# frozenreboot/rplidar_ros2_driver

Hardware: AMD Instinct MI355X
Metric: Mpoints/s raw-scan->filtered PointCloud2 (higher is better)
Workload: dtype u32/f32

## Files before the change

rplidar_ros2_driver_amd/csrc/rpl_device.hpp:

```cpp
#pragma once
#include <hip/hip_runtime.h>
#include <stdint.h>

#include "rplgpu.h"

namespace rpl {

constexpr int kBlock = 1024;
constexpr int kWaves = kBlock / 64;
constexpr int kIters = 32;
constexpr uint32_t kMaxN = 32768;
constexpr int kChunks = kIters * kWaves;
constexpr double kTwoPi = 6.283185307179586476925286766559;

struct Tables {
  const float *angle;
  const float *angle_inv;
  const float2 *cs;
  const float2 *cs_inv;
  const double *rcp;
  uint32_t *work_ctr;
  uint32_t n_cu;
  void *voxel_store;
  uint32_t voxel_store_wgs;
  uint32_t voxel_store_recs;
  unsigned long long *voxel_stats;
  unsigned long long *voxel_stats_host;
  int32_t voxel_split;
  const float *scan_t0;
  uint32_t *redo;
};

struct KParams {
  int32_t is_new_protocol;
  int32_t inverted;
  int32_t scan_processing;
  int32_t clip_enable;
  uint32_t q_min;
  float range_min;
  float range_max;
  float voxel_leaf;
  float ror_r2;
  uint32_t ror_k;
  double vox_scale;
  float vox_scale_f;
  int32_t vox_L;
  int32_t vox_bias;
  float inv_leaf;
  float leaf_s;
  float inv_leaf_s;
  uint32_t d_lo;
  uint32_t d_span;
  int32_t cell_range_safe;
  unsigned long long *dbg;
  uint32_t *cell_keys;
  int32_t fast_div;
  int32_t fast_d4000;
};

__device__ __forceinline__ uint32_t nd_q14(uint2 v) { return v.x & 0xFFFFu; }
__device__ __forceinline__ uint32_t nd_dist(uint2 v) {
  return __builtin_amdgcn_alignbit(v.y, v.x, 16);
}
__device__ __forceinline__ uint32_t nd_quality(uint2 v) { return (v.y >> 16) & 0xFFu; }

__device__ __forceinline__ float nd_dist_m(uint32_t dist_q2) {
  return __uint2float_rn(dist_q2) / 4000.0f;
}
__device__ __forceinline__ float nd_intensity(uint32_t quality, int is_new_protocol) {
  return is_new_protocol ? (float)quality : (float)(quality >> 2);
}
__device__ __forceinline__ bool nd_keep(uint32_t dist_q2, uint32_t quality, const KParams &p) {
  bool k = (dist_q2 - p.d_lo) <= p.d_span;
  if (p.clip_enable) k = k && (quality >= p.q_min);
// ... 100 lines not shown
```

rplidar_ros2_driver_amd/csrc/rpl_voxel.hip:

```cpp
#include <algorithm>
#include <cstdlib>
#include <type_traits>

#include "rpl_device.hpp"
#include "rpl_launch.hpp"
#include "rpl_xf.hpp"

namespace rpl {

#ifndef RPL_VOXEL_THREADS
#define RPL_VOXEL_THREADS 1024
#endif
#ifndef RPL_VOXEL_WGS_PER_CU
#define RPL_VOXEL_WGS_PER_CU (RPL_VOXEL_THREADS == 512 ? 2 : 1)
#endif
constexpr int kVB = RPL_VOXEL_THREADS;
constexpr int kVW = kVB / 64;
constexpr int kVWG = RPL_VOXEL_WGS_PER_CU;
constexpr uint32_t kRecCap = kVWG == 2 ? 4096u : 7168u;
constexpr uint32_t kRecPerThread = kRecCap / kVB;
constexpr uint32_t kRowCap = kVWG == 2 ? 1024u : 2u * kVB;
constexpr uint32_t kRowsPerThread = kRowCap / kVB;
constexpr uint32_t kBucketCap = kRecCap + 3u * kRowCap;
constexpr uint32_t kEmptyKey = 0xFFFFFFFFu;
// ... 242 lines not shown
  const u32x4 marker = {kEmptyKey, 0u, 0u, 0u};
  VoxelLds &L = S.L;
  uint4 *const G = S.G;
  const uint32_t lds_rec = (uint32_t)(uintptr_t)&L.rec[0];
  if (base + 1u + total <= kRecCap) {
    if (lane_id() == 0) lds_store128(lds_rec + base * 16u, marker);
#pragma unroll
    for (int j = 0; j < NS; ++j)
      if (__builtin_amdgcn_inverse_ballot_w64(m[j])) lds_store128(lds_rec + pos[j] * 16u, rec[j]);
  } else {
    if (lane_id() == 0) {
      if (base < kRecCap) lds_store128(lds_rec + base * 16u, marker); else glb_store128(G + base, marker);
    }
#pragma unroll
    for (int j = 0; j < NS; ++j) {
      if (__builtin_amdgcn_inverse_ballot_w64(m[j])) {
        if (pos[j] < kRecCap) lds_store128(lds_rec + pos[j] * 16u, rec[j]); else glb_store128(G + pos[j], rec[j]);
      }
    }
  }
  return false;
}

template <int NS>
__device__ __forceinline__ void voxel_block_split(QueueSink &S,
                                                  const bool (&ok)[NS], const uint32_t (&key)[NS],
                                                  const uint32_t (&qx)[NS], const uint32_t (&qy)[NS],
                                                  const uint32_t (&ci)[NS]) {
#pragma unroll
  for (uint32_t cls = 0; cls < 2u; ++cls) {
    bool okc[NS];
    uint32_t keyc[NS], qxc[NS], qyc[NS], cic[NS];
#pragma unroll
    for (int j = 0; j < NS; ++j) {
      okc[j] = ok[j] && (((key[j] >> 16) ^ key[j]) & 1u) == cls;
      keyc[j] = key[j];
      qxc[j] = okc[j] ? qx[j] : 0u;
      qyc[j] = okc[j] ? qy[j] : 0u;
      cic[j] = okc[j] ? ci[j] : 0u;
    }
    voxel_block_pass<true, NS, kPassPlain>(S, okc, keyc, qxc, qyc, cic);
  }
}

__device__ __forceinline__ double run_sum_f64(uint32_t u) {
  double s = (double)u;
  if (u >= 0xF0000000u) s -= 4294967296.0;
  return s;
}

struct VoxelArena {
  float4 *base;
  unsigned long long *cursor;
  unsigned long long capacity;
  unsigned long long *scan_start;
  int xyi;
};
enum : int { kEmitLegacy = 0, kEmitArenaFirst = 1, kEmitCountOnly = 2, kEmitArenaKnown = 3, kEmitArenaTemp = 4 };

template <bool DBG>
struct PhaseClock {
  unsigned long long acc[8] = {0, 0, 0, 0, 0, 0, 0, 0}, mark = 0;
  __device__ __forceinline__ void start() {
    if (DBG) mark = clock64();
  }
  __device__ __forceinline__ void lap(int i) {
    if (DBG) {
      const unsigned long long now = clock64();
      acc[i] += now - mark;
      mark = now;
    }
  }
};

template <bool DBG, bool CELLS>
__device__ __forceinline__ uint32_t voxel_reduce(VoxelLds &L, const KParams &p,
                                                 float4 *__restrict__ out, uint32_t out_stride,
                                                 uint32_t b, uint32_t *ncell_out, int mode,
                                                 const VoxelArena &arena, bool normalised,
                                                 const float4 *out_buffer) {
  PhaseClock<DBG> pc;
  pc.start();
  auto flush_dbg = [&]() {
    if (DBG && p.dbg && threadIdx.x == 0) {
#pragma unroll
      for (int i = 1; i < 8; ++i) atomicAdd(&p.dbg[16 * b + i], pc.acc[i]);
    }
  };
  uint32_t *const rowstart = L.rows, *const rowfill = L.rows + kRowCap;
  uint32_t *cell_keys = p.cell_keys ? p.cell_keys + (out - out_buffer) : nullptr;
  const int vbias = p.vox_bias;
  const uint32_t nrec = L.misc[0];
  if (DBG && p.dbg && threadIdx.x == 0) pc.acc[7] += (unsigned long long)nrec << 40;
  uint4 mine[kRecPerThread];
  uint32_t rmin = 0xFFFFFFFFu, rmax = 0u;
#pragma unroll
  for (int k = 0; k < (int)kRecPerThread; ++k) {
    const uint32_t idx = threadIdx.x + (uint32_t)k * kVB;
    uint4 m = make_uint4(kEmptyKey, 0u, 0u, 0u);
    if ((idx & ~63u) < nrec) {
      const uint4 raw = L.rec[idx];
      const bool ok = idx < nrec && raw.x != kEmptyKey;
      m = raw;
      if (!normalised) {
        uint4 pr;
        pr.y = (uint32_t)__builtin_amdgcn_update_dpp(0, (int)raw.y, 0x138, 0xF, 0xF, false);
// ... 831 lines not shown
        L.misc[7] = 0u;
      }
      __syncthreads();
      arena_at = ((unsigned long long)L.tmp[29] << 32) | L.tmp[28];
      out = arena.base + arena_at;
      emit_mode = kEmitArenaKnown;
    }
    if (emit_mode == kEmitArenaTemp && L.misc[3] == 0u) {
      const uint32_t total = L.misc[7];
      if (threadIdx.x == 0) {
        const unsigned long long at = atomicAdd(arena.cursor, (unsigned long long)total);
        L.tmp[28] = (uint32_t)at;
        L.tmp[29] = (uint32_t)(at >> 32);
      }
      __syncthreads();
      arena_at = ((unsigned long long)L.tmp[29] << 32) | L.tmp[28];
      const unsigned long long room = arena_at >= arena.capacity ? 0ull : arena.capacity - arena_at;
      const uint32_t ncopy = (uint32_t)min((unsigned long long)total, room);
      const float4 *src = reinterpret_cast<const float4 *>(G + T.voxel_store_recs);
      if (arena.xyi) {
        float *dst = reinterpret_cast<float *>(arena.base) + 3u * (size_t)arena_at;
        for (uint32_t i = threadIdx.x; i < ncopy; i += kVB) {
          const float4 v = src[i];
          dst[3u * i] = v.x;
          dst[3u * i + 1u] = v.y;
          dst[3u * i + 2u] = v.w;
        }
      } else {
        float4 *dst = arena.base + arena_at;
        for (uint32_t i = threadIdx.x; i < ncopy; i += kVB) dst[i] = src[i];
      }
    }
  }
  if (DBG && p.dbg && threadIdx.x == 0) {
    atomicAdd(&p.dbg[16 * b], pc.acc[0]);
    atomicAdd(&p.dbg[16 * b + 2], pc.acc[2]);
  }

  if (flags) atomicOr(&L.misc[1], flags);
  __syncthreads();
  if (threadIdx.x == 0 && !abandoned) {
    const uint32_t total = L.misc[7];
    if (arena.base) {
      const unsigned long long room = arena_at >= arena.capacity ? 0ull : arena.capacity - arena_at;
      const uint32_t kept = (uint32_t)min((unsigned long long)total, room);
      arena.scan_start[b] = arena_at;
      n_points[b] = kept;
      if (status) status[b] = L.misc[1] | (kept < total ? RPLGPU_SCAN_OUT_TRUNCATED : 0u);
    } else {
      n_points[b] = min(total, out_stride);
      if (status) status[b] = L.misc[1] | ((total > out_stride) ? RPLGPU_SCAN_OUT_TRUNCATED : 0u);
    }
  }
  if (RORM != 2 && B <= gridDim.x) return;
  if (threadIdx.x == 0) L.tmp[31] = gridDim.x + atomicAdd(&T.work_ctr[0], 1u);
  __syncthreads();
  bl = L.tmp[31];
  __syncthreads();
  }
}

template <bool FAST_DIV, bool SAFE, bool DBG, bool SPLIT, int RORM = 0>
__global__ __launch_bounds__(kVB) __attribute__((amdgpu_waves_per_eu(kVB * kVWG / 256, kVB * kVWG / 256))) void k_cloud_voxel(
    const uint2 *__restrict__ nodes, uint32_t n_stride, const uint32_t *__restrict__ n_per_scan,
    KParams p, Tables T, const uint32_t *__restrict__ keepmask, uint32_t mask_stride,
    float4 *__restrict__ xyzi, uint32_t out_stride, uint32_t *__restrict__ n_points,
    uint32_t *__restrict__ status, uint32_t B, VoxelArena arena, uint4 *__restrict__ store,
    uint32_t group, uint32_t n_scans, const float *__restrict__ motion,
    const float *__restrict__ pose2d) {
  __shared__ VoxelLds L;
  uint4 *G = store + (size_t)blockIdx.x * 2u * T.voxel_store_recs;
  const float2 *cs = p.inverted ? T.cs_inv : T.cs;
  const uint32_t ishift = p.is_new_protocol ? 0u : 2u;
  const uint32_t ibfe_off = 16u + ishift, ibfe_w = 0xFFu >> ishift;
  const uint32_t q_min16 = p.clip_enable ? (min(p.q_min, 256u) << 16) : 0u;
  const bool use_xf = (group > 1u) || motion || pose2d;
  __shared__ RorSide Rs;
  auto phase_s = [&](uint32_t b, uint32_t, uint32_t &flags) -> bool {
    QueueSink sink{L, G};
    const uint32_t s_lo = b * group, s_hi = min(n_scans, s_lo + group);
    for (uint32_t sc = s_lo; sc < s_hi; ++sc) {
      const uint32_t n = (uint32_t)__builtin_amdgcn_readfirstlane(
          (int)min(n_per_scan[sc], min(n_stride, kMaxN)));
      const uint2 *scan = nodes + (size_t)sc * n_stride;
      const __amdgpu_buffer_rsrc_t scan_rsrc =
          __builtin_amdgcn_make_buffer_rsrc((void *)scan, 0, (int)(n * 8u), 0x00020000);
      const ScanSide sd = scan_side(sc, keepmask, mask_stride, motion, pose2d, T.scan_t0);
      const uint32_t blk0 = (uint32_t)__builtin_amdgcn_readfirstlane((int)wave_id());
      if constexpr (RORM == 1) {
        if (threadIdx.x == 0) { Rs.n_todo = 0u; Rs.n_todo2 = 0u; }
        __syncthreads();
        voxel_stream_dispatch<FAST_DIV, SAFE, SPLIT, false, RPL_VOXEL_AHEAD, 1>(
            sink, p, cs, scan_rsrc, blk0, (n + 123u) / 124u, sd, 0u, use_xf, q_min16, ibfe_off, ibfe_w, flags,
            nullptr, &Rs, (n * 8u + 15u) & ~15u);
        asm volatile("s_waitcnt vmcnt(0) lgkmcnt(0)" ::: "memory");
        __syncthreads();
        bool clutter;
        if (use_xf)
          clutter = ror_resolve<FAST_DIV, SAFE, true>(sink, Rs, p, cs, scan, n, sd.xf, q_min16, ibfe_off, ibfe_w, flags);
        else
          clutter = ror_resolve<FAST_DIV, SAFE, false>(sink, Rs, p, cs, scan, n, sd.xf, q_min16, ibfe_off, ibfe_w, flags);
        if (clutter) return true;
        __syncthreads();
      } else {
        voxel_stream_dispatch<FAST_DIV, SAFE, SPLIT, DBG, RPL_VOXEL_AHEAD, RORM>(
            sink, p, cs, scan_rsrc, blk0, (n + 127u) >> 7, sd, mask_stride, use_xf, q_min16, ibfe_off,
            ibfe_w, flags, (DBG && p.dbg) ? p.dbg + 16 * b : nullptr);
      }
    }
    return false;
  };
  voxel_work_loop<DBG, RORM, SPLIT || RORM != 0>(L, p, T, G, xyzi, out_stride, n_points, status, B, 0u, arena, phase_s);
}

__global__ __launch_bounds__(256) void k_validate_div(float d, float rd, uint32_t e_lo,
                                                      uint32_t e_hi, uint32_t *mismatches) {
  const uint64_t per_exp = 1ull << 23;
  const uint64_t total = (uint64_t)(e_hi - e_lo + 1) * per_exp;
  uint32_t bad = 0;
  for (uint64_t t = (uint64_t)blockIdx.x * blockDim.x + threadIdx.x; t < total;
       t += (uint64_t)gridDim.x * blockDim.x) {
    uint32_t bits = ((uint32_t)(e_lo + (uint32_t)(t >> 23)) << 23) | (uint32_t)(t & (per_exp - 1));
    float a = __uint_as_float(bits);
    float na = __uint_as_float(bits | 0x80000000u);
    const f2 q2 = div_by2(f2{a, na}, d, rd);
    bad += (__float_as_uint(q2.x) != __float_as_uint(a / d));
    bad += (__float_as_uint(q2.y) != __float_as_uint(na / d));
    bad += (__float_as_uint(div_by(a, d, rd)) != __float_as_uint(a / d));
  }
  if (blockIdx.x == 0 && threadIdx.x == 0) {
    bad += (div_by(0.0f, d, rd) != 0.0f);
    bad += (div_by(-0.0f, d, rd) != 0.0f);
  }
  if (bad) atomicAdd(mismatches, bad);
}

hipError_t launch_validate_div(hipStream_t s, float d, float rd, uint32_t e_lo, uint32_t e_hi,
                               uint32_t *d_mismatches) {
  hipLaunchKernelGGL(k_validate_div, dim3(256 * 16), dim3(256), 0, s, d, rd, e_lo, e_hi,
                     d_mismatches);
  return hipGetLastError();
}

uint32_t voxel_max_workgroups(uint32_t n_cu) { return (uint32_t)kVWG * (n_cu ? n_cu : 256u); }


hipError_t launch_cloud_voxel(hipStream_t s, const void *nodes, uint32_t n_stride,
                              const uint32_t *n_per_scan, uint32_t B, const KParams &p,
                              const Tables &T, const uint32_t *keepmask, uint32_t mask_stride,
                              float *xyzi, uint32_t out_stride, uint32_t *n_points,
                              uint32_t *status, float *arena, unsigned long long arena_capacity,
                              unsigned long long *arena_cursor, unsigned long long *scan_start,
                              uint32_t group, const float *motion, const float *pose2d,
                              int arena_form, int ror_mode) {
  if (B == 0) return hipSuccess;
  if (ror_mode && (!p.fast_div || !T.redo || p.dbg)) return hipErrorInvalidValue;
  if (ror_mode == 2 && !keepmask) return hipErrorInvalidValue;
  if (arena_form == 2 && !ror_mode && (p.dbg || !T.voxel_split)) return hipErrorInvalidValue;
  if (group == 0) group = 1;
  group = std::min(group, B);
  const uint32_t n_scans = B;
  B = (B + group - 1u) / group;
  if (!T.voxel_store || T.voxel_store_wgs == 0) return hipErrorInvalidValue;
  if (voxel_store_need(group, n_stride) > T.voxel_store_recs) return hipErrorInvalidValue;
  VoxelArena ar;
  ar.base = (float4 *)arena;
  ar.cursor = arena_cursor;
  ar.capacity = arena_capacity;
  ar.scan_start = scan_start;
  ar.xyi = arena ? arena_form : 0;
  if (kVWG == 2 && group > 1) return hipErrorInvalidValue;
  uint32_t grid = std::min<uint32_t>(std::min<uint32_t>(B, voxel_max_workgroups(T.n_cu)),
                                     T.voxel_store_wgs);
  if (const char *e = std::getenv("RPLGPU_VOXEL_GRID")) {
    const long g = std::atol(e);
    if (g > 0) grid = std::min<uint32_t>(grid, (uint32_t)g);
  }
  const bool with_stats = T.voxel_stats && T.voxel_stats_host && B >= 64u && ror_mode != 2;
  Tables Tk = T;
  if (!with_stats) Tk.voxel_stats = nullptr;
  if (with_stats)
    if (hipError_t e = hipMemsetAsync(T.voxel_stats, 0, 16, s); e != hipSuccess) return e;
  if (grid < B || ror_mode == 2)
    if (hipError_t e = hipMemsetAsync(T.work_ctr, 0, 4, s); e != hipSuccess) return e;
#define RPL_LAUNCH_VOXEL(FD, SF, DB, SP)                                                          \
  hipLaunchKernelGGL((k_cloud_voxel<FD, SF, DB, SP>), dim3(grid), dim3(kVB), 0, s, (const uint2 *)nodes, \
                     n_stride, n_per_scan, p, Tk, keepmask, mask_stride, (float4 *)xyzi, out_stride, \
                     n_points, status, B, ar, (uint4 *)T.voxel_store, group, n_scans, motion, pose2d)
#define RPL_LAUNCH_VOXEL_SF(FD, DB, SP)                                                           \
  do {                                                                                             \
    if (p.cell_range_safe) RPL_LAUNCH_VOXEL(FD, true, DB, SP); else RPL_LAUNCH_VOXEL(FD, false, DB, SP); \
  } while (0)
#define RPL_LAUNCH_VOXEL_ROR(SF, SP, RM)                                                          \
  hipLaunchKernelGGL((k_cloud_voxel<true, SF, false, SP, RM>), dim3(grid), dim3(kVB), 0, s,         \
                     (const uint2 *)nodes, n_stride, n_per_scan, p, Tk, keepmask, mask_stride,      \
                     (float4 *)xyzi, out_stride, n_points, status, B, ar, (uint4 *)T.voxel_store,   \
                     group, n_scans, motion, pose2d)
#define RPL_LAUNCH_VOXEL_ROR_SF(SP, RM)                                                           \
  do {                                                                                             \
    if (p.cell_range_safe) RPL_LAUNCH_VOXEL_ROR(true, SP, RM); else RPL_LAUNCH_VOXEL_ROR(false, SP, RM); \
  } while (0)
  if (ror_mode == 1) {
    if (T.voxel_split) RPL_LAUNCH_VOXEL_ROR_SF(true, 1); else RPL_LAUNCH_VOXEL_ROR_SF(false, 1);
  } else if (ror_mode == 2) {
    if (T.voxel_split) RPL_LAUNCH_VOXEL_ROR_SF(true, 2); else RPL_LAUNCH_VOXEL_ROR_SF(false, 2);
  } else
  if (p.dbg) {
    if (p.fast_div) RPL_LAUNCH_VOXEL_SF(true, true, false); else RPL_LAUNCH_VOXEL_SF(false, true, false);
  } else if (T.voxel_split) {
    if (p.fast_div) RPL_LAUNCH_VOXEL_SF(true, false, true); else RPL_LAUNCH_VOXEL_SF(false, false, true);
  } else {
    if (p.fast_div) RPL_LAUNCH_VOXEL_SF(true, false, false); else RPL_LAUNCH_VOXEL_SF(false, false, false);
  }
#undef RPL_LAUNCH_VOXEL_SF
#undef RPL_LAUNCH_VOXEL
#undef RPL_LAUNCH_VOXEL_ROR_SF
#undef RPL_LAUNCH_VOXEL_ROR
  if (with_stats) {
    if (hipError_t e = hipMemcpyAsync(T.voxel_stats_host, T.voxel_stats, 16, hipMemcpyDeviceToHost, s);
        e != hipSuccess)
      return e;
  }
  return hipGetLastError();
}

}
```

rplidar_ros2_driver_amd/csrc/rplgpu_api.hip:

```cpp
#include <hip/hip_runtime.h>
#include <dlfcn.h>

#include <algorithm>
#include <cmath>
#include <cstdio>
#include <cstdlib>
#include <cstring>
#include <limits>
#include <new>
#include <string>
#include <thread>
#include <vector>

#include "rplgpu.h"
#include "rplgpu_msg.h"
#include "rpl_launch.hpp"
#include "rpl_msg.hpp"
#include "rpl_comm_layout.hpp"
#include "rpl_cells.hpp"

struct VoxelBatchId {
  const void *nodes = nullptr;
  uint32_t n_stride = 0, B = 0, group = 0;
  bool operator==(const VoxelBatchId &o) const {
    return nodes == o.nodes && n_stride == o.n_stride && B == o.B && group == o.group;
  }
};

struct rplgpu_ctx {
  int device = -1;
  hipStream_t own_stream = nullptr;
  hipStream_t stream = nullptr;
  uint32_t max_n = 0, max_b = 0;
  float *d_angle = nullptr, *d_angle_inv = nullptr, *d_inc = nullptr, *d_rinc = nullptr;
  float2 *d_cs = nullptr, *d_cs_inv = nullptr;
  double *d_rcp = nullptr;
  unsigned char *h_pin = nullptr;
  unsigned char *d_pin = nullptr;
  bool zero_copy = true;
  bool spin_sync = true;
  size_t flag_off = 0;
  uint32_t scan_seq = 0;
  struct Pinned { unsigned char *host, *dev; size_t bytes; };
  std::vector<Pinned> pinned;
  unsigned char *d_nodes = nullptr, *d_out = nullptr;
  uint32_t *d_rormask = nullptr;
  uint32_t *d_redo = nullptr;
  int32_t ror_fused = 1;
  uint32_t *d_need_sort = nullptr;
  uint32_t need_sort_cap = 0;
  uint32_t *d_small = nullptr;
  bool div4000_ok = false;
  float leaf_checked = 0.0f;
  bool leaf_ok = false;
  bool idx_checked = false, idx_ok = false;
  unsigned long long *dbg = nullptr;
  uint32_t *cell_keys = nullptr;
  const float *scan_t0 = nullptr;
  unsigned long long *h_vstats = nullptr;
  uint32_t stats_group = 1;
  bool stats_valid = false;
  VoxelBatchId stats_id;
  struct VoxelDecision { VoxelBatchId id; bool split = false; bool valid = false; };
  VoxelDecision decisions[8];
  uint32_t next_decision = 0;
  int32_t last_split = 0;
  uint32_t n_cu = 0;
  void *d_vstore = nullptr;
  int32_t force_split = -1;
  bool dec_stage = true;
  uint32_t vstore_wgs = 0;
  uint32_t vstore_recs = 0;
  uint32_t *d_merge = nullptr;
  size_t merge_cap = 0;
  unsigned long long *d_mkeys = nullptr;
  size_t mkeys_cap = 0;
  bool mkeys_clean = true;
  float2 *d_medges = nullptr;
  size_t medges_cap = 0;
  bool mspec_valid = false;
  rplgpu_scan_merge_t mspec;
  rpl::MergeK mspec_k;
  unsigned char *d_dec = nullptr;
  size_t dec_cap = 0;
  unsigned char *d_scans = nullptr;
  size_t scans_cap = 0;
  uint32_t *d_dec_todo = nullptr;
  size_t dec_todo_cap = 0;
  bool check_ptrs = true;
  void *comm = nullptr;
  int32_t comm_rank = 0, comm_world = 0;
  hipStream_t xstream = nullptr;
  hipEvent_t ev_main = nullptr, ev_x[4] = {nullptr, nullptr, nullptr, nullptr};
  uint32_t n_exchanges = 0;
  std::string err;
};

struct rplgpu_nccl_id_t {
  char internal[128];
};

namespace {

constexpr uint32_t kMaskStride = rpl::kMaxN / 32u;
constexpr size_t kTail = 64;

thread_local std::string g_create_err;

#define RPL_HIP(ctx, call)                                                              \
  do {                                                                                  \
    hipError_t e_ = (call);                                                             \
    if (e_ != hipSuccess) {                                                             \
      (ctx)->err = std::string(#call) + ": " + hipGetErrorString(e_);                   \
      return RPLGPU_ERR_HIP;                                                            \
    }                                                                                   \
  } while (0)

inline float host_dist_m(uint32_t d) { return static_cast<float>(d) / 4000.0f; }

bool make_keep_interval(float range_min, float range_max, uint32_t *lo, uint32_t *hi) {
  const uint32_t dmax = 0xFFFFFFFFu;
  if (!(host_dist_m(dmax) >= range_min)) return false;
  if (!(host_dist_m(1u) <= range_max)) return false;
  uint32_t a = 1u, b = dmax;
  while (a < b) {
    uint32_t m = a + (b - a) / 2;
    if (host_dist_m(m) >= range_min) b = m; else a = m + 1;
  }
  *lo = a;
  a = 1u, b = dmax;
  while (a < b) {
    uint32_t m = a + (b - a + 1) / 2;
    if (host_dist_m(m) <= range_max) a = m; else b = m - 1;
  }
  *hi = a;
  return *lo <= *hi;
}

rpl::KParams to_kparams(const rplgpu_params_t &p) {
  rpl::KParams k;
  k.is_new_protocol = p.is_new_protocol != 0;
  k.inverted = p.inverted != 0;
  k.scan_processing = p.scan_processing != 0;
  k.clip_enable = p.clip_enable != 0;
  k.q_min = p.q_min;
  k.range_min = p.range_min;
  k.range_max = p.range_max;
  k.voxel_leaf = p.voxel_leaf;
  k.ror_r2 = p.ror_radius * p.ror_radius;
  k.ror_k = p.ror_min_neighbors;
  k.vox_scale = 1.0;
  k.vox_scale_f = 1.0f;
  k.vox_L = 1;
  k.vox_bias = 0;
  k.inv_leaf = 1.0f;
  k.leaf_s = 1.0f;
  k.inv_leaf_s = 1.0f;
  k.fast_div = 0;
  k.fast_d4000 = 0;
  k.dbg = nullptr;
  k.cell_keys = nullptr;
  k.d_lo = 1u;
  k.d_span = 0xFFFFFFFEu;
  k.cell_range_safe = 0;
  if (k.clip_enable) {
    uint32_t lo, hi;
// ... 14 lines not shown
    k.inv_leaf = 1.0f / p.voxel_leaf;
    k.leaf_s = p.voxel_leaf * k.vox_scale_f;
    k.inv_leaf_s = k.inv_leaf / k.vox_scale_f;
  }
  return k;
}

bool voxel_split_for(rplgpu_ctx *c, const void *d_nodes, uint32_t n_stride, uint32_t B, uint32_t group) {
  group = std::max(1u, std::min(group, std::max(B, 1u)));
  const VoxelBatchId id{d_nodes, n_stride, B, group};
  const bool with_stats = c->h_vstats && (B + group - 1u) / group >= 64u;
  auto find = [&](const VoxelBatchId &k) -> rplgpu_ctx::VoxelDecision * {
    for (auto &d : c->decisions)
      if (d.valid && d.id == k) return &d;
    return nullptr;
  };
  if (c->h_vstats && c->stats_valid) {
    const unsigned long long entries = __atomic_load_n(&c->h_vstats[0], __ATOMIC_RELAXED);
    const unsigned long long items = __atomic_load_n(&c->h_vstats[1], __ATOMIC_RELAXED);
    const uint32_t g = c->stats_group;
    if (items != 0 && entries <= items * g * 70000ull) {
      rplgpu_ctx::VoxelDecision *d = find(c->stats_id);
      if (!d) {
        d = &c->decisions[c->next_decision];
        c->next_decision = (c->next_decision + 1u) % (uint32_t)(sizeof(c->decisions) / sizeof(c->decisions[0]));
        d->id = c->stats_id;
        d->split = false;
        d->valid = true;
      }
      const unsigned long long avg = entries / (items * g);
      if (!d->split && avg > 6500ull) d->split = true;
      else if (d->split && avg < 4000ull) d->split = false;
    }
  }
  const rplgpu_ctx::VoxelDecision *mine = find(id);
  const bool split = mine ? mine->split : false;
  if (with_stats) {
    c->stats_id = id;
    c->stats_valid = true;
    c->stats_group = group;
  }
  c->last_split = (c->force_split >= 0 ? c->force_split != 0 : split) ? 1 : 0;
  return c->last_split != 0;
}

rpl::Tables tables_of(rplgpu_ctx *c) {
  rpl::Tables t;
  t.angle = c->d_angle;
  t.angle_inv = c->d_angle_inv;
  t.cs = c->d_cs;
  t.cs_inv = c->d_cs_inv;
  t.rcp = c->d_rcp;
  t.work_ctr = c->d_small + 16;
  t.n_cu = c->n_cu;
  t.voxel_store = c->d_vstore;
  t.voxel_store_wgs = c->vstore_wgs;
  t.voxel_store_recs = c->vstore_recs;
  t.voxel_stats = reinterpret_cast<unsigned long long *>(c->d_small + 24);
  t.voxel_stats_host = c->h_vstats;
  t.voxel_split = c->force_split > 0 ? 1 : 0;
  t.scan_t0 = c->scan_t0;
  t.redo = c->d_redo;
  return t;
}

void build_tables(std::vector<float> &angle, std::vector<float> &angle_inv,
                  std::vector<float2> &cs, std::vector<float2> &cs_inv, std::vector<float> &inc,
                  std::vector<float> &rinc) {
  angle.resize(65536);
  angle_inv.resize(65536);
  cs.resize(65536);
  cs_inv.resize(65536);
  for (int q = 0; q < 65536; ++q) {
    uint16_t angle_z_q14 = (uint16_t)q;
    float angle_deg = angle_z_q14 * 90.0f / 16384.0f;
    float angle_rad = angle_deg * (M_PI / 180.0f);
    if (angle_rad < 0.0f) angle_rad += 2.0f * M_PI;
    if (angle_rad >= 2.0f * M_PI) angle_rad -= 2.0f * M_PI;
    float inv = (2.0f * M_PI) - angle_rad;
    if (inv >= 2.0f * M_PI) inv -= 2.0f * M_PI;
    angle[q] = angle_rad;
    angle_inv[q] = inv;
    cs[q] = make_float2((float)std::cos((double)angle_rad), (float)std::sin((double)angle_rad));
    cs_inv[q] = make_float2((float)std::cos((double)inv), (float)std::sin((double)inv));
  }
  inc.resize(rpl::kMaxN + 1);
  inc[0] = 0.0f;
  for (uint32_t c = 1; c <= rpl::kMaxN; ++c)
    inc[c] = static_cast<float>((2.0 * M_PI) / static_cast<double>(c));
  rinc.resize(rpl::kMaxN + 1);
  rinc[0] = 0.0f;
  for (uint32_t c = 1; c <= rpl::kMaxN; ++c) rinc[c] = 1.0f / inc[c];
}

template <class T>
int32_t upload(rplgpu_ctx *c, T **dst, const std::vector<T> &src) {
  RPL_HIP(c, hipMalloc((void **)dst, src.size() * sizeof(T)));
  RPL_HIP(c, hipMemcpy(*dst, src.data(), src.size() * sizeof(T), hipMemcpyHostToDevice));
  return RPLGPU_OK;
}

void comm_teardown(rplgpu_ctx *c);

void free_ctx(rplgpu_ctx *c) {
  if (!c) return;
  if (c->device >= 0) (void)hipSetDevice(c->device);
// ... 222 lines not shown
  if (const char *e = std::getenv("RPLGPU_CHECK_POINTERS")) c->check_ptrs = std::atoi(e) != 0;
  auto fail = [&](int32_t code) {
    g_create_err = c->err;
    free_ctx(c);
    return code;
  };
  if (hipStreamCreateWithFlags(&c->own_stream, hipStreamNonBlocking) != hipSuccess)
    return fail(RPLGPU_ERR_HIP);
  c->stream = c->own_stream;

  std::vector<float> angle, angle_inv, inc, rinc;
  std::vector<float2> cs, cs_inv;
  build_tables(angle, angle_inv, cs, cs_inv, inc, rinc);
  for (int q = 1; q < 65536; ++q) {
    if (!(angle[q] > angle[q - 1])) {
      c->err = "angle table not strictly increasing";
      return fail(RPLGPU_ERR_INVALID_ARG);
    }
  }
  std::vector<double> rcp(rpl::kMaxN + 1);
  rcp[0] = 0.0;
  for (uint32_t k = 1; k <= rpl::kMaxN; ++k) rcp[k] = 1.0 / static_cast<double>(k);
  int32_t rc;
  if ((rc = upload(c, &c->d_rcp, rcp)) || (rc = upload(c, &c->d_angle, angle)) || (rc = upload(c, &c->d_angle_inv, angle_inv)) ||
      (rc = upload(c, &c->d_cs, cs)) || (rc = upload(c, &c->d_cs_inv, cs_inv)) ||
      (rc = upload(c, &c->d_inc, inc)) || (rc = upload(c, &c->d_rinc, rinc)))
    return fail(rc);

  const size_t n = c->max_n;
  c->flag_off = n * 8 + n * 16 + 2 * kTail;
  if (hipHostMalloc((void **)&c->h_pin, n * 8 + n * 16 + 3 * kTail, hipHostMallocDefault) != hipSuccess ||
      hipMalloc((void **)&c->d_nodes, n * 8 + kTail) != hipSuccess ||
      hipMalloc((void **)&c->d_out, n * 16 + kTail) != hipSuccess ||
      hipMalloc((void **)&c->d_small, 128) != hipSuccess ||
      hipMalloc((void **)&c->d_need_sort, ((size_t)c->max_b + 1u) * 4u) != hipSuccess ||
      hipMalloc((void **)&c->d_rormask, (size_t)c->max_b * kMaskStride * 4u) != hipSuccess ||
      hipMalloc((void **)&c->d_redo, ((size_t)c->max_b + 4u) * 4u) != hipSuccess) {
    c->err = "staging allocation failed";
    return fail(RPLGPU_ERR_HIP);
  }
  c->need_sort_cap = c->max_b;
  if (hipMemset(c->d_need_sort, 0, 4) != hipSuccess) {
    c->err = "staging allocation failed";
    return fail(RPLGPU_ERR_HIP);
  }
  c->vstore_wgs = std::min<uint32_t>(c->max_b, rpl::voxel_max_workgroups(c->n_cu));
  c->vstore_recs = (uint32_t)rpl::voxel_store_need(1u, rpl::kMaxN);
  if (hipMalloc(&c->d_vstore, (size_t)c->vstore_wgs * c->vstore_recs * 32u) != hipSuccess) {
    c->err = "record store allocation failed";
    return fail(RPLGPU_ERR_HIP);
  }
  if (hipHostMalloc((void **)&c->h_vstats, 16, hipHostMallocDefault) == hipSuccess) {
    c->h_vstats[0] = c->h_vstats[1] = 0ull;
  } else {
    c->h_vstats = nullptr;
    (void)hipGetLastError();
  }
  if (hipHostGetDevicePointer((void **)&c->d_pin, c->h_pin, 0) != hipSuccess) c->d_pin = nullptr;
  if (const char *e = std::getenv("RPLGPU_ZERO_COPY")) c->zero_copy = std::atoi(e) != 0;
  if (!c->d_pin) c->zero_copy = false;
  if (const char *e = std::getenv("RPLGPU_SPIN_SYNC")) c->spin_sync = std::atoi(e) != 0;
  if (const char *e = std::getenv("RPLGPU_DEC_STAGE")) c->dec_stage = std::atoi(e) != 0;
  if (const char *e = std::getenv("RPLGPU_VOXEL_SPLIT")) c->force_split = std::atoi(e) != 0;
  if (const char *e = std::getenv("RPLGPU_ROR_FUSED")) c->ror_fused = std::atoi(e) != 0;
  std::memset(c->h_pin + c->flag_off, 0, kTail);
  if (hipMemset(c->d_small, 0, 128) != hipSuccess) {
    c->err = "staging clear failed";
    return fail(RPLGPU_ERR_HIP);
  }
  if (validate_divisor(c, 4000.0f, 127, 159, &c->div4000_ok) != RPLGPU_OK) return fail(RPLGPU_ERR_HIP);
  if (validate_divisor(c, 0.05f, 27, 167, &c->leaf_ok) != RPLGPU_OK) return fail(RPLGPU_ERR_HIP);
  c->leaf_checked = 0.05f;
  *out = c;
  return RPLGPU_OK;
}

int32_t rplgpu_destroy(rplgpu_handle_t h) {
  if (!h) return RPLGPU_ERR_INVALID_ARG;
  (void)hipSetDevice(h->device);
  (void)hipStreamSynchronize(h->stream);
  free_ctx(h);
  return RPLGPU_OK;
}

const char *rplgpu_last_error(rplgpu_handle_t h) {
  if (!h) return g_create_err.c_str();
  return h->err.c_str();
}

int32_t rplgpu_set_stream(rplgpu_handle_t h, void *hip_stream) {
  if (!h) return RPLGPU_ERR_INVALID_ARG;
  hipStream_t next = hip_stream ? (hipStream_t)hip_stream : h->own_stream;
  if (next != h->stream) {
    RPL_HIP(h, hipSetDevice(h->device));
    RPL_HIP(h, hipStreamSynchronize(h->stream));
  }
  h->stream = next;
  return RPLGPU_OK;
}

int32_t rplgpu_set_cell_key_output(rplgpu_handle_t h, uint32_t *d_cell_keys) {
  if (!h) return RPLGPU_ERR_INVALID_ARG;
  if (d_cell_keys && !device_readable(h, d_cell_keys, "d_cell_keys")) return RPLGPU_ERR_INVALID_ARG;
  h->cell_keys = d_cell_keys;
  return RPLGPU_OK;
}

int32_t rplgpu_set_scan_time_offsets_dev(rplgpu_handle_t h, const float *d_t0) {
  if (!h) return RPLGPU_ERR_INVALID_ARG;
  if (d_t0 && !device_readable(h, d_t0, "d_t0")) return RPLGPU_ERR_INVALID_ARG;
  h->scan_t0 = d_t0;
  return RPLGPU_OK;
}

int32_t rplgpu_set_voxel_aggregation(rplgpu_handle_t h, int32_t mode) {
  if (!h || mode < RPLGPU_VOXEL_AGG_AUTO || mode > RPLGPU_VOXEL_AGG_TWO_CLASS) return RPLGPU_ERR_INVALID_ARG;
  h->force_split = mode == RPLGPU_VOXEL_AGG_AUTO ? -1 : (mode == RPLGPU_VOXEL_AGG_TWO_CLASS ? 1 : 0);
  return RPLGPU_OK;
}

int32_t rplgpu_debug_set_cycle_buffer(rplgpu_handle_t h, void *d_buf) {
  if (!h) return RPLGPU_ERR_INVALID_ARG;
  h->dbg = (unsigned long long *)d_buf;
  return RPLGPU_OK;
}
int32_t rplgpu_debug_ascend_sorted(rplgpu_handle_t h, uint32_t *count) {
  if (!h || !count) return RPLGPU_ERR_INVALID_ARG;
  RPL_HIP(h, hipSetDevice(h->device));
  RPL_HIP(h, hipStreamSynchronize(h->stream));
  RPL_HIP(h, hipMemcpy(count, h->d_small + 28, 4, hipMemcpyDeviceToHost));
  return RPLGPU_OK;
}
int32_t rplgpu_debug_voxel_instance(rplgpu_handle_t h) { return h ? h->last_split : RPLGPU_ERR_INVALID_ARG; }
int32_t rplgpu_set_ror_mode(rplgpu_handle_t h, int32_t mode) {
  if (!h || (mode != RPLGPU_ROR_INSIDE && mode != RPLGPU_ROR_TWO_KERNELS)) return RPLGPU_ERR_INVALID_ARG;
  h->ror_fused = mode == RPLGPU_ROR_INSIDE ? 1 : 0;
  return RPLGPU_OK;
}
int32_t rplgpu_debug_ror_listed(rplgpu_handle_t h, uint32_t *count) {
  if (!h || !count) return RPLGPU_ERR_INVALID_ARG;
  RPL_HIP(h, hipSetDevice(h->device));
  RPL_HIP(h, hipStreamSynchronize(h->stream));
  RPL_HIP(h, hipMemcpy(count, h->d_redo, 4, hipMemcpyDeviceToHost));
  return RPLGPU_OK;
}
int32_t rplgpu_debug_fast_div(rplgpu_handle_t h) {
  if (!h) return RPLGPU_ERR_INVALID_ARG;
  return (h->div4000_ok ? 1 : 0) | (h->leaf_ok ? 2 : 0) | (h->idx_ok ? 4 : 0);
// ... 78 lines not shown
    if (ror_inside && h->ror_fused && p->voxel_enable && kp.fast_div && !kp.dbg) {
      *ror_inside = true;
    } else {
      RPL_HIP(h, rpl::launch_ror_mask(h->stream, d_nodes, n_stride, d_n_per_scan, B, kp,
                                      tables_of(h), h->d_rormask, kMaskStride));
      *mask_out = h->d_rormask;
    }
  }
  *kp_out = kp;
  return RPLGPU_OK;
}

constexpr uint32_t kRorListed = rpl::kRorListedBit;
static int32_t voxel_with_ror(rplgpu_handle_t h, const rplgpu_node_t *d_nodes, uint32_t n_stride,
                              const uint32_t *d_n_per_scan, uint32_t B, const rpl::KParams &kp,
                              const rpl::Tables &T, uint32_t *d_n_points, uint32_t *d_status,
                              float *d_arena, uint64_t arena_capacity, uint64_t *d_cursor,
                              uint64_t *d_start, uint32_t group, const float *d_motion,
                              const float *d_pose2d, int form, float *d_xyzi = nullptr,
                              uint32_t out_stride = 0, bool defer_listed = false) {
  RPL_HIP(h, hipMemsetAsync(h->d_redo, 0, 4, h->stream));
  RPL_HIP(h, rpl::launch_cloud_voxel(h->stream, d_nodes, n_stride, d_n_per_scan, B, kp, T, nullptr,
                                     kMaskStride, d_xyzi, out_stride, d_n_points, d_status, d_arena,
                                     arena_capacity, reinterpret_cast<unsigned long long *>(d_cursor),
                                     reinterpret_cast<unsigned long long *>(d_start), group, d_motion,
                                     d_pose2d, form, 1));
  if (defer_listed) return RPLGPU_OK;
  RPL_HIP(h, rpl::launch_ror_mask(h->stream, d_nodes, n_stride, d_n_per_scan, B, kp, T, h->d_rormask,
                                  kMaskStride, true, std::max(1u, std::min(group, B))));
  RPL_HIP(h, rpl::launch_cloud_voxel(h->stream, d_nodes, n_stride, d_n_per_scan, B, kp, T, h->d_rormask,
                                     kMaskStride, d_xyzi, out_stride, d_n_points, d_status, d_arena,
                                     arena_capacity, reinterpret_cast<unsigned long long *>(d_cursor),
                                     reinterpret_cast<unsigned long long *>(d_start), group, d_motion,
                                     d_pose2d, form, 2));
  return RPLGPU_OK;
}

static int32_t cloud_arena_impl(rplgpu_handle_t h, const rplgpu_node_t *d_nodes, uint32_t n_stride,
                               const uint32_t *d_n_per_scan, uint32_t B, const rplgpu_params_t *p,
                               float *d_arena, uint64_t arena_capacity, uint64_t *d_cursor,
                               uint64_t *d_scan_start, uint32_t *d_n_points, uint32_t *d_status,
                               bool xyi) {
  int32_t rc = check_batch(h, d_nodes, n_stride, d_n_per_scan, B);
  if (rc) return rc;
  if (!p || !d_arena || !d_cursor || !d_scan_start || !d_n_points) return RPLGPU_ERR_INVALID_ARG;
  if (!p->voxel_enable) {
    h->err = "rplgpu_cloud_arena_dev needs voxel_enable";
    return RPLGPU_ERR_INVALID_ARG;
  }
  rpl::KParams kp;
  const uint32_t *mask = nullptr;
  bool ror_inside = false;
  if ((rc = prepare_cloud(h, d_nodes, n_stride, d_n_per_scan, B, p, &kp, &mask, &ror_inside))) return rc;
  RPL_HIP(h, hipMemsetAsync(d_cursor, 0, 8, h->stream));
  static_assert(sizeof(unsigned long long) == sizeof(uint64_t), "64-bit cursor");
  rpl::Tables T_arena = tables_of(h);
  T_arena.voxel_split = voxel_split_for(h, d_nodes, n_stride, B, 1u) ? 1 : 0;
  if (ror_inside)
    return voxel_with_ror(h, d_nodes, n_stride, d_n_per_scan, B, kp, T_arena, d_n_points, d_status, d_arena,
                          arena_capacity, d_cursor, d_scan_start, 1u, nullptr, nullptr, xyi ? 1 : 0);
  RPL_HIP(h, rpl::launch_cloud_voxel(h->stream, d_nodes, n_stride, d_n_per_scan, B, kp,
                                     T_arena, mask, kMaskStride, nullptr, 0, d_n_points,
                                     d_status, d_arena, arena_capacity,
                                     reinterpret_cast<unsigned long long *>(d_cursor),
                                     reinterpret_cast<unsigned long long *>(d_scan_start), 1u, nullptr,
                                     nullptr, xyi ? 1 : 0));
  return RPLGPU_OK;
}

int32_t rplgpu_cloud_arena_dev(rplgpu_handle_t h, const rplgpu_node_t *d_nodes, uint32_t n_stride,
                               const uint32_t *d_n_per_scan, uint32_t B, const rplgpu_params_t *p,
                               float *d_arena, uint64_t arena_capacity, uint64_t *d_cursor,
                               uint64_t *d_scan_start, uint32_t *d_n_points, uint32_t *d_status) {
  return cloud_arena_impl(h, d_nodes, n_stride, d_n_per_scan, B, p, d_arena, arena_capacity, d_cursor,
                          d_scan_start, d_n_points, d_status, false);
}

int32_t rplgpu_cloud_arena_xyi_dev(rplgpu_handle_t h, const rplgpu_node_t *d_nodes,
                                   uint32_t n_stride, const uint32_t *d_n_per_scan, uint32_t B,
                                   const rplgpu_params_t *p, float *d_slot, uint64_t slot_points,
                                   uint64_t *d_cursor, uint64_t *d_scan_start, uint32_t *d_n_points,
                                   uint32_t *d_status) {
  return cloud_arena_impl(h, d_nodes, n_stride, d_n_per_scan, B, p, d_slot, slot_points, d_cursor,
                          d_scan_start, d_n_points, d_status, true);
}

static int32_t fused_impl(rplgpu_handle_t h, const rplgpu_node_t *d_nodes, uint32_t n_stride,
                          const uint32_t *d_n_per_scan, uint32_t B, uint32_t group,
                          const rplgpu_params_t *p, const float *d_motion, const float *d_pose2d,
                          float *d_arena, uint64_t arena_capacity, uint64_t *d_cursor,
                          uint64_t *d_group_start, uint32_t *d_n_points, uint32_t *d_status,
                          bool cells) {
  int32_t rc = check_batch(h, d_nodes, n_stride, d_n_per_scan, B);
  if (rc) return rc;
  if (!p || !d_arena || !d_cursor || !d_group_start || !d_n_points || group == 0)
    return RPLGPU_ERR_INVALID_ARG;
  if (!p->voxel_enable) {
    h->err = cells ? "rplgpu_cloud_fused_cells_dev needs voxel_enable" : "rplgpu_cloud_fused_voxel_dev needs voxel_enable";
    return RPLGPU_ERR_INVALID_ARG;
  }
  if ((d_motion && !device_readable(h, d_motion, "d_motion")) ||
      (d_pose2d && !device_readable(h, d_pose2d, "d_pose2d")))
    return RPLGPU_ERR_INVALID_ARG;
  if (h->scan_t0 && !d_motion) {
    h->err = "rplgpu_cloud_fused_voxel_dev: scan time offsets are set (rplgpu_set_scan_time_offsets_dev) but d_motion is NULL";
    return RPLGPU_ERR_INVALID_ARG;
  }
  group = std::min(group, B);
  const uint64_t need = rpl::voxel_store_need(group, n_stride);
  if (need > h->vstore_recs) {
    if (need > (1ull << 24)) {
      h->err = "rplgpu_cloud_fused_voxel_dev: group x n_stride above 2^24 samples";
      return RPLGPU_ERR_CAPACITY;
    }
    RPL_HIP(h, hipSetDevice(h->device));
    RPL_HIP(h, hipStreamSynchronize(h->stream));
    void *bigger = nullptr;
    if (hipMalloc(&bigger, (size_t)h->vstore_wgs * need * 32u) != hipSuccess) {
      h->err = "record store allocation failed";
      (void)hipGetLastError();
      return RPLGPU_ERR_HIP;
    }
    (void)hipFree(h->d_vstore);
    h->d_vstore = bigger;
    h->vstore_recs = (uint32_t)need;
  }
  rpl::KParams kp;
  const uint32_t *mask = nullptr;
  bool ror_inside = false;
  if ((rc = prepare_cloud(h, d_nodes, n_stride, d_n_per_scan, B, p, &kp, &mask, &ror_inside))) return rc;
  if (cells) {
    kp.cell_keys = nullptr;
    kp.dbg = nullptr;
  }
  RPL_HIP(h, hipMemsetAsync(d_cursor, 0, 8, h->stream));
  rpl::Tables T_fused = tables_of(h);
  T_fused.voxel_split = voxel_split_for(h, d_nodes, n_stride, B, group) ? 1 : 0;
  const int form = cells ? 2 : 0;
  if (ror_inside)
    return voxel_with_ror(h, d_nodes, n_stride, d_n_per_scan, B, kp, T_fused, d_n_points, d_status, d_arena,
                          arena_capacity, d_cursor, d_group_start, group, d_motion, d_pose2d, form);
  if (cells) T_fused.voxel_split = 1;
  RPL_HIP(h, rpl::launch_cloud_voxel(h->stream, d_nodes, n_stride, d_n_per_scan, B, kp,
                                     T_fused, mask, kMaskStride, nullptr, 0, d_n_points,
                                     d_status, d_arena, arena_capacity,
                                     reinterpret_cast<unsigned long long *>(d_cursor),
                                     reinterpret_cast<unsigned long long *>(d_group_start), group,
                                     d_motion, d_pose2d, form));
  return RPLGPU_OK;
}

int32_t rplgpu_cloud_fused_voxel_dev(rplgpu_handle_t h, const rplgpu_node_t *d_nodes,
                                     uint32_t n_stride, const uint32_t *d_n_per_scan, uint32_t B,
                                     uint32_t group, const rplgpu_params_t *p,
                                     const float *d_motion, const float *d_pose2d, float *d_arena,
                                     uint64_t arena_capacity, uint64_t *d_cursor,
                                     uint64_t *d_group_start, uint32_t *d_n_points,
                                     uint32_t *d_status) {
  return fused_impl(h, d_nodes, n_stride, d_n_per_scan, B, group, p, d_motion, d_pose2d, d_arena,
                    arena_capacity, d_cursor, d_group_start, d_n_points, d_status, false);
}

int32_t rplgpu_cloud_fused_cells_dev(rplgpu_handle_t h, const rplgpu_node_t *d_nodes,
                                     uint32_t n_stride, const uint32_t *d_n_per_scan, uint32_t B,
                                     uint32_t group, const rplgpu_params_t *p,
                                     const float *d_motion, const float *d_pose2d,
                                     rplgpu_cell_t *d_cells, uint64_t cells_capacity,
                                     uint64_t *d_cursor, uint64_t *d_group_start,
                                     uint32_t *d_n_cells, uint32_t *d_status) {
  return fused_impl(h, d_nodes, n_stride, d_n_per_scan, B, group, p, d_motion, d_pose2d,
                    reinterpret_cast<float *>(d_cells), cells_capacity, d_cursor, d_group_start, d_n_cells,
                    d_status, true);
}


int32_t rplgpu_scan_merge_edges(const rplgpu_scan_merge_t *m, float *edges, float *inc) {
  if (!m) return RPLGPU_ERR_INVALID_ARG;
  if (!std::isfinite(m->angle_min) || !std::isfinite(m->angle_max) || !std::isfinite(m->range_min) ||
      !std::isfinite(m->range_max) || !std::isfinite(m->scan_time))
    return RPLGPU_ERR_INVALID_ARG;
  if (m->count == 0 || m->count > RPLGPU_MAX_MERGE_BEAMS) return RPLGPU_ERR_INVALID_ARG;
  const double span = (double)m->angle_max - (double)m->angle_min;
  const float f_inc = (float)(span / (double)m->count);
  if (!(f_inc > 0.0f) || f_inc > (float)(M_PI / 2)) return RPLGPU_ERR_INVALID_ARG;
  if (span > 2.0 * M_PI * (1.0 + 0x1p-20)) return RPLGPU_ERR_INVALID_ARG;
  if (!(0.0f <= m->range_min && m->range_min < m->range_max)) return RPLGPU_ERR_INVALID_ARG;
  if (edges)
    for (uint32_t k = 0; k <= m->count; ++k) {
      const double phi = (double)m->angle_min + (double)k * (double)f_inc;
      edges[2 * k] = (float)std::cos(phi);
      edges[2 * k + 1] = (float)std::sin(phi);
// ... 1645 lines not shown
```

Baseline: 295,400.

## Reset voxel counters in-kernel via last-block epilogue instead of host memsets

Removes the per-launch hipMemsetAsync calls for the work counter, arena cursor and stats, and the stats D2H copy. The last workgroup to finish, found through a new done counter, now publishes the cursor and stats (stats go to pinned host memory) and resets the counters for the next call. A host-side 'clean' flag tracks whether the counters are known to be zero, so the voxel pipeline can become a single kernel command. The cost is extra atomics and fences at kernel exit, plus correctness risk if a launch aborts or the stream changes.

```diff
diff --git a/rplidar_ros2_driver_amd/csrc/rpl_device.hpp b/rplidar_ros2_driver_amd/csrc/rpl_device.hpp
--- a/rplidar_ros2_driver_amd/csrc/rpl_device.hpp
+++ b/rplidar_ros2_driver_amd/csrc/rpl_device.hpp
@@ -20,6 +20,10 @@
   const float2 *cs_inv;
   const double *rcp;
   uint32_t *work_ctr;
+  uint32_t *done_ctr;
+  unsigned long long *arena_cursor;
+  unsigned long long *voxel_stats_dev;
+  bool *counters_clean;
   uint32_t n_cu;
   void *voxel_store;
   uint32_t voxel_store_wgs;
diff --git a/rplidar_ros2_driver_amd/csrc/rpl_voxel.hip b/rplidar_ros2_driver_amd/csrc/rpl_voxel.hip
--- a/rplidar_ros2_driver_amd/csrc/rpl_voxel.hip
+++ b/rplidar_ros2_driver_amd/csrc/rpl_voxel.hip
@@ -318,6 +318,7 @@
 struct VoxelArena {
   float4 *base;
   unsigned long long *cursor;
+  unsigned long long *cursor_out;
   unsigned long long capacity;
   unsigned long long *scan_start;
   int xyi;
@@ -1255,11 +1256,29 @@
       if (status) status[b] = L.misc[1] | ((total > out_stride) ? RPLGPU_SCAN_OUT_TRUNCATED : 0u);
     }
   }
-  if (RORM != 2 && B <= gridDim.x) return;
+  if (RORM != 2 && B <= gridDim.x) break;
   if (threadIdx.x == 0) L.tmp[31] = gridDim.x + atomicAdd(&T.work_ctr[0], 1u);
   __syncthreads();
   bl = L.tmp[31];
   __syncthreads();
+  }
+  if constexpr (RORM == 0) {
+    if (T.done_ctr && threadIdx.x == 0) {
+      __threadfence();
+      if (atomicAdd(T.done_ctr, 1u) == gridDim.x - 1u) {
+        __threadfence();
+        if (T.voxel_stats) {
+          const unsigned long long entries = atomicExch(&T.voxel_stats[0], 0ull);
+          const unsigned long long items = atomicExch(&T.voxel_stats[1], 0ull);
+          __hip_atomic_store(&T.voxel_stats_dev[0], entries, __ATOMIC_RELAXED, __HIP_MEMORY_SCOPE_SYSTEM);
+          __hip_atomic_store(&T.voxel_stats_dev[1], items, __ATOMIC_RELAXED, __HIP_MEMORY_SCOPE_SYSTEM);
+        }
+        if (arena.cursor_out) *arena.cursor_out = atomicExch(arena.cursor, 0ull);
+        atomicExch(T.work_ctr, 0u);
+        atomicExch(T.done_ctr, 0u);
+        __threadfence_system();
+      }
+    }
   }
 }
 
@@ -1356,23 +1375,30 @@
                               unsigned long long *arena_cursor, unsigned long long *scan_start,
                               uint32_t group, const float *motion, const float *pose2d,
                               int arena_form, int ror_mode) {
-  if (B == 0) return hipSuccess;
-  if (ror_mode && (!p.fast_div || !T.redo || p.dbg)) return hipErrorInvalidValue;
-  if (ror_mode == 2 && !keepmask) return hipErrorInvalidValue;
-  if (arena_form == 2 && !ror_mode && (p.dbg || !T.voxel_split)) return hipErrorInvalidValue;
+  const bool owns_cursor = arena && arena_cursor && ror_mode == 0;
+  auto nothing_launched = [&](hipError_t why) {
+    if (owns_cursor)
+      if (hipError_t e = hipMemsetAsync(arena_cursor, 0, 8, s); e != hipSuccess && why == hipSuccess) return e;
+    return why;
+  };
+  if (B == 0) return nothing_launched(hipSuccess);
+  if (ror_mode && (!p.fast_div || !T.redo || p.dbg)) return nothing_launched(hipErrorInvalidValue);
+  if (ror_mode == 2 && !keepmask) return nothing_launched(hipErrorInvalidValue);
+  if (arena_form == 2 && !ror_mode && (p.dbg || !T.voxel_split)) return nothing_launched(hipErrorInvalidValue);
   if (group == 0) group = 1;
   group = std::min(group, B);
   const uint32_t n_scans = B;
   B = (B + group - 1u) / group;
-  if (!T.voxel_store || T.voxel_store_wgs == 0) return hipErrorInvalidValue;
-  if (voxel_store_need(group, n_stride) > T.voxel_store_recs) return hipErrorInvalidValue;
+  if (!T.voxel_store || T.voxel_store_wgs == 0) return nothing_launched(hipErrorInvalidValue);
+  if (voxel_store_need(group, n_stride) > T.voxel_store_recs) return nothing_launched(hipErrorInvalidValue);
   VoxelArena ar;
   ar.base = (float4 *)arena;
   ar.cursor = arena_cursor;
+  ar.cursor_out = nullptr;
   ar.capacity = arena_capacity;
   ar.scan_start = scan_start;
   ar.xyi = arena ? arena_form : 0;
-  if (kVWG == 2 && group > 1) return hipErrorInvalidValue;
+  if (kVWG == 2 && group > 1) return nothing_launched(hipErrorInvalidValue);
   uint32_t grid = std::min<uint32_t>(std::min<uint32_t>(B, voxel_max_workgroups(T.n_cu)),
                                      T.voxel_store_wgs);
   if (const char *e = std::getenv("RPLGPU_VOXEL_GRID")) {
@@ -1380,12 +1406,39 @@
     if (g > 0) grid = std::min<uint32_t>(grid, (uint32_t)g);
   }
   const bool with_stats = T.voxel_stats && T.voxel_stats_host && B >= 64u && ror_mode != 2;
+  const bool with_queue = grid < B || ror_mode == 2;
   Tables Tk = T;
   if (!with_stats) Tk.voxel_stats = nullptr;
-  if (with_stats)
-    if (hipError_t e = hipMemsetAsync(T.voxel_stats, 0, 16, s); e != hipSuccess) return e;
-  if (grid < B || ror_mode == 2)
-    if (hipError_t e = hipMemsetAsync(T.work_ctr, 0, 4, s); e != hipSuccess) return e;
+  const bool one_command = ror_mode == 0 && T.done_ctr && T.arena_cursor && T.counters_clean &&
+                           (!with_stats || T.voxel_stats_dev);
+  bool stats_by_copy = false, cleared = false;
+  if (one_command) {
+    if (with_stats || with_queue || arena) {
+      if (!*T.counters_clean) {
+        if (hipError_t e = hipMemsetAsync(T.work_ctr, 0, 4, s); e != hipSuccess) return e;
+        if (hipError_t e = hipMemsetAsync(T.done_ctr, 0, 4, s); e != hipSuccess) return e;
+        if (hipError_t e = hipMemsetAsync(T.arena_cursor, 0, 8, s); e != hipSuccess) return e;
+        if (hipError_t e = hipMemsetAsync(T.voxel_stats, 0, 16, s); e != hipSuccess) return e;
+        cleared = true;
+      }
+      if (arena) {
+        ar.cursor = T.arena_cursor;
+        ar.cursor_out = arena_cursor;
+      }
+    } else {
+      Tk.done_ctr = nullptr;
+    }
+  } else {
+    Tk.done_ctr = nullptr;
+    if (T.counters_clean && (with_stats || with_queue)) *T.counters_clean = false;
+    if (arena && ror_mode == 0)
+      if (hipError_t e = hipMemsetAsync(arena_cursor, 0, 8, s); e != hipSuccess) return e;
+    if (with_stats)
+      if (hipError_t e = hipMemsetAsync(T.voxel_stats, 0, 16, s); e != hipSuccess) return e;
+    if (with_queue)
+      if (hipError_t e = hipMemsetAsync(T.work_ctr, 0, 4, s); e != hipSuccess) return e;
+    stats_by_copy = with_stats;
+  }
 #define RPL_LAUNCH_VOXEL(FD, SF, DB, SP)                                                          \
   hipLaunchKernelGGL((k_cloud_voxel<FD, SF, DB, SP>), dim3(grid), dim3(kVB), 0, s, (const uint2 *)nodes, \
                      n_stride, n_per_scan, p, Tk, keepmask, mask_stride, (float4 *)xyzi, out_stride, \
@@ -1419,12 +1472,14 @@
 #undef RPL_LAUNCH_VOXEL
 #undef RPL_LAUNCH_VOXEL_ROR_SF
 #undef RPL_LAUNCH_VOXEL_ROR
-  if (with_stats) {
+  if (stats_by_copy) {
     if (hipError_t e = hipMemcpyAsync(T.voxel_stats_host, T.voxel_stats, 16, hipMemcpyDeviceToHost, s);
         e != hipSuccess)
       return e;
   }
-  return hipGetLastError();
-}
-
-}
+  const hipError_t e = hipGetLastError();
+  if (e == hipSuccess && cleared) *T.counters_clean = true;
+  return e;
+}
+
+}
diff --git a/rplidar_ros2_driver_amd/csrc/rplgpu_api.hip b/rplidar_ros2_driver_amd/csrc/rplgpu_api.hip
--- a/rplidar_ros2_driver_amd/csrc/rplgpu_api.hip
+++ b/rplidar_ros2_driver_amd/csrc/rplgpu_api.hip
@@ -50,6 +50,7 @@
   uint32_t *d_need_sort = nullptr;
   uint32_t need_sort_cap = 0;
   uint32_t *d_small = nullptr;
+  bool vox_clean = false;
   bool div4000_ok = false;
   float leaf_checked = 0.0f;
   bool leaf_ok = false;
@@ -58,6 +59,7 @@
   uint32_t *cell_keys = nullptr;
   const float *scan_t0 = nullptr;
   unsigned long long *h_vstats = nullptr;
+  unsigned long long *d_vstats_pin = nullptr;
   uint32_t stats_group = 1;
   bool stats_valid = false;
   VoxelBatchId stats_id;
@@ -112,6 +114,7 @@
     hipError_t e_ = (call);                                                             \
     if (e_ != hipSuccess) {                                                             \
       (ctx)->err = std::string(#call) + ": " + hipGetErrorString(e_);                   \
+      (ctx)->vox_clean = false;               \
       return RPLGPU_ERR_HIP;                                                            \
     }                                                                                   \
   } while (0)
@@ -232,6 +235,10 @@
   t.cs_inv = c->d_cs_inv;
   t.rcp = c->d_rcp;
   t.work_ctr = c->d_small + 16;
+  t.done_ctr = c->d_small + 17;
+  t.arena_cursor = reinterpret_cast<unsigned long long *>(c->d_small + 18);
+  t.voxel_stats_dev = c->d_vstats_pin;
+  t.counters_clean = &c->vox_clean;
   t.n_cu = c->n_cu;
   t.voxel_store = c->d_vstore;
   t.voxel_store_wgs = c->vstore_wgs;
@@ -560,6 +567,10 @@
   }
   if (hipHostMalloc((void **)&c->h_vstats, 16, hipHostMallocDefault) == hipSuccess) {
     c->h_vstats[0] = c->h_vstats[1] = 0ull;
+    if (hipHostGetDevicePointer((void **)&c->d_vstats_pin, c->h_vstats, 0) != hipSuccess) {
+      c->d_vstats_pin = nullptr;
+      (void)hipGetLastError();
+    }
   } else {
     c->h_vstats = nullptr;
     (void)hipGetLastError();
@@ -602,6 +613,7 @@
   if (next != h->stream) {
     RPL_HIP(h, hipSetDevice(h->device));
     RPL_HIP(h, hipStreamSynchronize(h->stream));
+    h->vox_clean = false;
   }
   h->stream = next;
   return RPLGPU_OK;
@@ -786,10 +798,10 @@
   const uint32_t *mask = nullptr;
   bool ror_inside = false;
   if ((rc = prepare_cloud(h, d_nodes, n_stride, d_n_per_scan, B, p, &kp, &mask, &ror_inside))) return rc;
-  RPL_HIP(h, hipMemsetAsync(d_cursor, 0, 8, h->stream));
   static_assert(sizeof(unsigned long long) == sizeof(uint64_t), "64-bit cursor");
   rpl::Tables T_arena = tables_of(h);
   T_arena.voxel_split = voxel_split_for(h, d_nodes, n_stride, B, 1u) ? 1 : 0;
+  if (ror_inside) RPL_HIP(h, hipMemsetAsync(d_cursor, 0, 8, h->stream));
   if (ror_inside)
     return voxel_with_ror(h, d_nodes, n_stride, d_n_per_scan, B, kp, T_arena, d_n_points, d_status, d_arena,
                           arena_capacity, d_cursor, d_scan_start, 1u, nullptr, nullptr, xyi ? 1 : 0);
@@ -867,10 +879,10 @@
     kp.cell_keys = nullptr;
     kp.dbg = nullptr;
   }
-  RPL_HIP(h, hipMemsetAsync(d_cursor, 0, 8, h->stream));
   rpl::Tables T_fused = tables_of(h);
   T_fused.voxel_split = voxel_split_for(h, d_nodes, n_stride, B, group) ? 1 : 0;
   const int form = cells ? 2 : 0;
+  if (ror_inside) RPL_HIP(h, hipMemsetAsync(d_cursor, 0, 8, h->stream));
   if (ror_inside)
     return voxel_with_ror(h, d_nodes, n_stride, d_n_per_scan, B, kp, T_fused, d_n_points, d_status, d_arena,
                           arena_capacity, d_cursor, d_group_start, group, d_motion, d_pose2d, form);
```

New measurement: 297,300 (median of 6 runs). About the same (+0.6%).
